# Intelligent-Microsystems-Lab/SNNQuantPrune

Hardware: AMD Instinct MI355X
Metric: samples/sec/node (DVS128 T=20, 4-bit/90%-pruned) (higher is better)
Workload: dtype fp6*fp4->f32 (integer-exact); 1 GPU; C3 topology: 3x(qconv3x3+BN+LIF+pool2) + qdense(32768->110)+LIF + vote, DVS128 128x128x2, T=20, bits 4/4/4/4, 90% pruned; batch_per_gpu=1024, global_batch=1024, frames=20, parallelism=dp1 (batch-sharded, all-gather logits)

## Files before the change

### include/snnqp.h

```cpp
#ifndef SNNQP_H_
#define SNNQP_H_

#include <stdint.h>

#ifdef __cplusplus
extern "C" {
#endif

typedef void *snnqp_stream_t;

enum {
  SNNQP_OK = 0,
  SNNQP_EINVAL = -1,
  SNNQP_EUNSUPPORTED = -2,
  SNNQP_EHIP = -3
};

enum { SNNQP_F32 = 0, SNNQP_U8 = 1, SNNQP_BITS = 2, SNNQP_EV1 = 3, SNNQP_EV4 = 4 };
enum { SNNQP_W_F32 = 0, SNNQP_W_I8 = 1 };
enum {
  SNNQP_NEURON_NONE = 0,
  SNNQP_NEURON_MULTI_STEP_LIF = 1,
  SNNQP_NEURON_PARAMETRIC_LEAKY_IF = 2,
  SNNQP_NEURON_LIF = 3
// ... 59 lines not shown
  int32_t H, W, Cin, Cout;
  int32_t KH, KW;
  int32_t stride_h, stride_w;
  int32_t pad_h_lo, pad_h_hi, pad_w_lo, pad_w_hi;
  int32_t in_dil_h, in_dil_w;
  int32_t k_dil_h, k_dil_w;
  int32_t groups;
} snnqp_conv_geom_t;

typedef struct {
  int32_t D, H, W, Cin, Cout;
  int32_t KD, KH, KW;
  int32_t stride[3];
  int32_t pad_lo[3], pad_hi[3];
  int32_t in_dil[3];
  int32_t k_dil[3];
  int32_t groups;
} snnqp_conv3d_geom_t;

#define SNNQP_VERSION 505
int snnqp_version(void);
const char *snnqp_last_error(void);
const char *snnqp_build_flags(void);

int snnqp_conv_out_shape(const snnqp_conv_geom_t *g, int32_t *OH, int32_t *OW);

int snnqp_quantize(int kind, const float *w, const float *mask, int64_t n,
                   int bits, float p0, float p1, float *fq_out,
                   int8_t *codes_out, int32_t *flags, snnqp_stream_t stream);
int snnqp_quantize_ex(int kind, const float *w, const float *mask, int64_t n,
                      int bits, int sign, float p0, float p1, float *fq_out,
                      int8_t *codes_out, int32_t *flags, snnqp_stream_t stream);

int snnqp_pack_codes_mfma(const int8_t *w, int64_t K, int32_t N, int32_t Npad,
                          int8_t *wt, snnqp_stream_t stream);

int snnqp_pack_codes_fp6(const int8_t *w, int64_t K, int32_t N, int32_t Npad, void *wt6,
                         snnqp_stream_t stream);

int snnqp_inspect_f32(const float *x, int64_t n, int32_t *flags,
                      snnqp_stream_t stream);
int snnqp_inspect_u8(const uint8_t *x, int64_t n, int32_t *flags,
                     snnqp_stream_t stream);
int snnqp_f32_to_u8(const float *x, uint8_t *y, int64_t n,
                    snnqp_stream_t stream);
int snnqp_narrow_f32(const float *x, uint8_t *y, int64_t n, int32_t *flags,
// ... 176 lines not shown
```

### snnquantprune_amd/_lib.py

```python

from __future__ import annotations

import ctypes
import os
from ctypes import (POINTER, Structure, c_char_p, c_float, c_int, c_int8,
                    c_int32, c_uint32, c_int64, c_void_p)

_HERE = os.path.dirname(os.path.abspath(__file__))
LIB_PATH = os.path.join(_HERE, "csrc", "libsnnqp.so")

ABI_VERSION = 505

F32, U8, BITS, EV1, EV4 = 0, 1, 2, 3, 4
W_F32, W_I8 = 0, 1
NEURON_NONE, NEURON_MULTI_STEP_LIF, NEURON_PARAMETRIC_LEAKY_IF, NEURON_LIF = 0, 1, 2, 3
SURR_FAST_SIGMOID, SURR_ATAN, SURR_SLAYER, SURR_SMOOTH_STEP, SURR_PIECEWISE_LINEAR = 0, 1, 2, 3, 4
Q_DUQ, Q_UNIFORM_STATIC, Q_PARAMETRIC_D, Q_PARAMETRIC_D_XMAX = 0, 1, 2, 3
IMPL_AUTO, IMPL_GENERIC, IMPL_MFMA = 0, 1, 2
FLAG_CODE_OVERFLOW, FLAG_MASK_NOT_BINARY = 1, 2
FLAG_NOT_INTEGER, FLAG_GT_ONE, FLAG_GT_127, FLAG_GT_15 = 4, 8, 16, 32
OK, EINVAL, EUNSUPPORTED, EHIP = 0, -1, -2, -3
STATUS_QUEUE_CORRUPT, STATUS_TICKET, STATUS_BOUND = 1, 2, 4


# ... 13 lines not shown

class NeuronT(Structure):
  _fields_ = [("kind", c_int32), ("k", c_float), ("v_threshold", c_float),
              ("v_reset", c_float), ("decay", c_void_p)]


class ConvGeomT(Structure):
  _fields_ = [(n, c_int32) for n in (
      "H", "W", "Cin", "Cout", "KH", "KW", "stride_h", "stride_w",
      "pad_h_lo", "pad_h_hi", "pad_w_lo", "pad_w_hi",
      "in_dil_h", "in_dil_w", "k_dil_h", "k_dil_w", "groups")]


class Conv3dGeomT(Structure):
  _fields_ = ([(n, c_int32) for n in ("D", "H", "W", "Cin", "Cout", "KD", "KH", "KW")]
              + [(n, c_int32 * 3) for n in ("stride", "pad_lo", "pad_hi", "in_dil", "k_dil")]
              + [("groups", c_int32)])


_PROTOTYPES = {
    "snnqp_version": (c_int, []),
    "snnqp_last_error": (c_char_p, []),
    "snnqp_build_flags": (c_char_p, []),
    "snnqp_conv_out_shape": (c_int, [POINTER(ConvGeomT), POINTER(c_int32),
                                     POINTER(c_int32)]),
    "snnqp_quantize": (c_int, [c_int, c_void_p, c_void_p, c_int64, c_int, c_float,
                               c_float, c_void_p, c_void_p, c_void_p, c_void_p]),
    "snnqp_quantize_ex": (c_int, [c_int, c_void_p, c_void_p, c_int64, c_int, c_int, c_float,
                                  c_float, c_void_p, c_void_p, c_void_p, c_void_p]),
    "snnqp_pack_codes_mfma": (c_int, [c_void_p, c_int64, c_int32, c_int32, c_void_p,
                                      c_void_p]),
    "snnqp_pack_codes_fp6": (c_int, [c_void_p, c_int64, c_int32, c_int32, c_void_p, c_void_p]),
    "snnqp_inspect_f32": (c_int, [c_void_p, c_int64, c_void_p, c_void_p]),
    "snnqp_inspect_u8": (c_int, [c_void_p, c_int64, c_void_p, c_void_p]),
    "snnqp_f32_to_u8": (c_int, [c_void_p, c_void_p, c_int64, c_void_p]),
    "snnqp_narrow_f32": (c_int, [c_void_p, c_void_p, c_int64, c_void_p, c_void_p]),
    "snnqp_pack_frames": (c_int, [c_void_p, c_int64, c_int32, c_int32, c_int, c_void_p, c_void_p,
                                  c_void_p]),
    "snnqp_unpack_frames": (c_int, [c_void_p, c_int, c_int64, c_int32, c_int32, c_void_p,
                                    c_void_p]),
    "snnqp_pack_bits": (c_int, [c_void_p, c_int, c_int64, c_int32, c_void_p,
                                c_void_p]),
    "snnqp_pack_bits_checked": (c_int, [c_void_p, c_int, c_int64, c_int32, c_void_p, c_void_p,
                                        c_void_p]),
    "snnqp_unpack_bits": (c_int, [c_void_p, c_int64, c_int32, c_void_p, c_void_p]),
    "snnqp_conv_forward": (c_int, [c_void_p, c_int, c_int64, POINTER(ConvGeomT),
# ... 143 lines not shown
```

### snnquantprune_amd/csrc/api.hip

```cpp
#include "common.h"

namespace snnqp {

static thread_local std::string g_last_error;

void set_error(const char *fmt, ...) {
  char buf[512];
  va_list ap;
  va_start(ap, fmt);
  vsnprintf(buf, sizeof(buf), fmt, ap);
  va_end(ap);
  g_last_error = buf;
}

}

extern "C" {

int snnqp_version(void) { return SNNQP_VERSION; }

const char *snnqp_last_error(void) { return snnqp::g_last_error.c_str(); }

#ifndef SNNQP_BUILD_FLAGS
#define SNNQP_BUILD_FLAGS ""
#endif
const char *snnqp_build_flags(void) { return SNNQP_BUILD_FLAGS; }

int snnqp_conv_out_shape(const snnqp_conv_geom_t *g, int32_t *OH, int32_t *OW) {
  SNNQP_REQUIRE(g && OH && OW, SNNQP_EINVAL, "conv_out_shape: null argument");
  SNNQP_REQUIRE(g->stride_h > 0 && g->stride_w > 0 && g->in_dil_h > 0 &&
                    g->in_dil_w > 0 && g->k_dil_h > 0 && g->k_dil_w > 0 &&
                    g->KH > 0 && g->KW > 0,
                SNNQP_EINVAL, "conv_out_shape: non-positive stride/dilation/kernel");
  const int64_t hd = g->H > 0 ? (int64_t)(g->H - 1) * g->in_dil_h + 1 : 0;
  const int64_t wd = g->W > 0 ? (int64_t)(g->W - 1) * g->in_dil_w + 1 : 0;
  const int64_t kh = (int64_t)(g->KH - 1) * g->k_dil_h + 1;
  const int64_t kw = (int64_t)(g->KW - 1) * g->k_dil_w + 1;
  const int64_t th = hd + g->pad_h_lo + g->pad_h_hi;
  const int64_t tw = wd + g->pad_w_lo + g->pad_w_hi;
  *OH = th < kh ? 0 : (int32_t)((th - kh) / g->stride_h + 1);
  *OW = tw < kw ? 0 : (int32_t)((tw - kw) / g->stride_w + 1);
  return SNNQP_OK;
}

}
```

### snnquantprune_amd/csrc/conv3x3_bits.hip

```cpp
#include <type_traits>

#include "conv_tile.h"

namespace snnqp {

typedef int v8i __attribute__((ext_vector_type(8)));
typedef float v16f __attribute__((ext_vector_type(16)));
typedef __attribute__((address_space(3))) const v4i lds_cv4i_t;
typedef __attribute__((address_space(3))) const uint32_t lds_cu32_t;

constexpr int F6_PITCH = HPITCH;
constexpr int F6_ROWS = 6;
constexpr int F6_NT = 256;
constexpr int F6_PLANE = F6_ROWS * HPITCH * 32;
constexpr int F6_NBUF = 3;
constexpr int F6_TAB = 256 * 32 * 4;
constexpr int DQT_BYTES = 16384;

__device__ __forceinline__ uint32_t fp6_codes4(uint32_t x) {
  const uint32_t m1 = (x >> 7) & 0x01010101u;
  const uint32_t mag = (x ^ (m1 * 0xFFu)) + m1;
  const uint32_t code = __builtin_amdgcn_perm(0x1E1C1A18u, 0x14100800u, mag);
  return code | (m1 << 5);
}

__device__ __forceinline__ uint32_t squeeze6(uint32_t c) {
  return (c & 0x3Fu) | ((c >> 2) & 0xFC0u) | ((c >> 4) & 0x3F000u) | ((c >> 6) & 0xFC0000u);
}

__device__ __forceinline__ void fp6_pack32(const v4i &lo, const v4i &hi, int (&d)[6]) {
  uint32_t t[8];
#pragma unroll
  for (int i = 0; i < 4; ++i) {
    t[i] = squeeze6(fp6_codes4((uint32_t)lo[i]));
    t[4 + i] = squeeze6(fp6_codes4((uint32_t)hi[i]));
  }
#pragma unroll
  for (int g = 0; g < 2; ++g) {
    d[3 * g + 0] = (int)(t[4 * g] | (t[4 * g + 1] << 24));
    d[3 * g + 1] = (int)((t[4 * g + 1] >> 8) | (t[4 * g + 2] << 16));
    d[3 * g + 2] = (int)((t[4 * g + 2] >> 16) | (t[4 * g + 3] << 8));
  }
}

enum { FMT_FP6 = 0, FMT_I8 = 1 };

constexpr int F6_WR_SLOT = 2;
constexpr int F6_BAR_SLOT = 4;
constexpr int F6_PF = 4;

__host__ __device__ constexpr int pair_tap(int p, int h) { return p < 3 ? p + 3 * h : 2 * p + h; }

template <int FMT, int CIN, int NF, bool POOL, int DQ, bool FMA = false, bool BNF = false, bool BNU = false>
__global__ void __launch_bounds__(F6_NT, 2)
conv3x3_bits_kernel(ConvMfmaArgs a) {
  static_assert(CIN == 32 || CIN == 64 || CIN == 96 || CIN == 128, "one to four 32-channel groups");
  static_assert(!BNU || (BNF && DQ == DQ_TABLE), "the uniform multiplier folds into the shared table");
  static_assert(DQ == DQ_ARITH || DQ == DQ_ONE || DQ == DQ_TABLE, "dequantisation mode");
  constexpr bool I8 = FMT == FMT_I8;
  constexpr bool TABLE = DQ == DQ_TABLE;
  static_assert(!(TABLE && I8), "the table is addressed by a float32 accumulator");
  typedef typename std::conditional<I8, v16i, v16f>::type acc_t;
  constexpr int BR = I8 ? 4 : 6;
  constexpr int WPP = CIN / 32;
  constexpr int NP = I8 ? WPP : (WPP + 1) / 2;
  constexpr int NPL = I8 ? WPP : WPP / 2;
  constexpr int PAIRS = I8 || WPP % 2 == 0 ? 0 : 5;
  constexpr int KS = 9 * NPL + PAIRS;
  constexpr int NPD = NPL > 0 ? NPL : 1;
  constexpr int HALO_B = NP * F6_PLANE;
  constexpr int FL = POOL ? 16 : 4;
  constexpr int SLOTS = 2 * FL;
  constexpr int NPIX = OutStage<POOL>::NPIX / 2;
  constexpr int TAB_OFF = F6_NBUF * HALO_B;
  constexpr int OB_OFF = TAB_OFF + (I8 ? 0 : F6_TAB);
  constexpr int DQT_OFF = OB_OFF + SLOTS * NPIX * 16 + 16;
  __shared__ __attribute__((aligned(128))) uint8_t lds[DQT_OFF + (TABLE ? DQT_BYTES : 0)];
  uint32_t *nxt = (uint32_t *)(lds + OB_OFF + SLOTS * NPIX * 16);
  uint32_t *obuf = (uint32_t *)(lds + OB_OFF);
  const uint32_t lds0 = lds_addr(lds) & 0x3FFFFu;

  const int tid = threadIdx.x, lane = tid & 63, wave = tid >> 6;
  const int n = lane & 31, h = lane >> 5;
  const int cg = wave & 3;
  const int cout_base = blockIdx.y * 128 + cg * 32;
  const bool wave_on = cout_base < a.Cout;
  const int cout = wave_on ? cout_base + n : n;
  const int cpar = cout < a.Cout ? cout : a.Cout - 1;
  const uint32_t cmask = chan_mask(cout_base, a.Cout);

  if (!I8) {
    for (int i = tid; i < 256 * 32; i += F6_NT) {
      const int e = i >> 5;
      uint32_t v = 0;
#pragma unroll
      for (int bit = 0; bit < 8; ++bit) v |= ((e >> bit) & 1) ? (0x2u << (4 * bit)) : 0u;
      ((uint32_t *)(lds + TAB_OFF))[i] = v;
    }
  }
  int bf[KS][BR];
  {
    const v4i *wtile = (const v4i *)a.wt + (int64_t)(cout_base >> 5) * (9 * WPP) * 64;
#pragma unroll
    for (int ks = 0; ks < KS; ++ks) {
      if constexpr (I8) {
        const v4i t = wave_on ? wtile[ks * 64 + lane] : v4i{0, 0, 0, 0};
        bf[ks][0] = t.x; bf[ks][1] = t.y; bf[ks][2] = t.z; bf[ks][3] = t.w;
      } else {
        const int ptap = pair_tap(ks - 9 * NPL, h);
        const bool pair = ks >= 9 * NPL;
        const int ks8 = pair ? ptap * WPP + WPP - 1 : (ks / NPD) * WPP + (ks % NPD) * 2 + h;
        v4i lo = {0, 0, 0, 0}, hi = {0, 0, 0, 0};
        if (wave_on && !(pair && ptap >= 9)) {
          lo = wtile[ks8 * 64 + n];
          hi = wtile[ks8 * 64 + 32 + n];
        }
        fp6_pack32(lo, hi, bf[ks]);
      }
    }
  }

  const uint32_t dqt_mid = lds0 + (uint32_t)DQT_OFF + 4u * (uint32_t)(TABLE ? a.lut_bound : 0);
  const float chain0 = TABLE ? __uint_as_float(dqt_mid) : 0.0f;
  if (TABLE) {
    const float mul0 = (BNU && a.bn.mul) ? a.bn.mul[0] : 1.0f;
    for (int i = tid; i <= 2 * a.lut_bound; i += F6_NT) {
      const float af = (float)(i - a.lut_bound);
      const float q = __builtin_fmaf(af, a.dq.rL, af * a.dq.rLlo);
      const float cur = q * a.dq.m;
      ((float *)(lds + DQT_OFF))[i] = BNU ? cur * mul0 : cur;
    }
  }

  LaneConsts lc = {0.f, 1.f, 0.f, 0.f, a.nrn.vr};
  if (a.bn.mean) { lc.bmean = a.bn.mean[cpar]; lc.bmul = a.bn.mul[cpar]; lc.bbias = a.bn.bias[cpar]; }
  if (a.nrn.kind == SNNQP_NEURON_LIF) lc.dec = a.nrn.decay[cpar];

  constexpr int SCALE_A = TABLE ? 64 : 127;
  constexpr int SCALE_B = TABLE ? 43 : 127;

  const int ty = ((n >> 2) & 1) | ((n >> 4) << 1);
  const int tx = (n & 3) | (((n >> 3) & 1) << 2);
  const uint32_t pixb = lds0 + (uint32_t)((ty * F6_PITCH + tx) * 32);
  const uint32_t abase_even = pixb + (uint32_t)((h ^ (ty & 1)) * 16);
  const uint32_t abase_odd = pixb + (uint32_t)((h ^ (ty & 1) ^ 1) * 16);
  const uint32_t abase_pv = pixb + (uint32_t)(h * F6_PITCH * 32 + ((ty ^ h) & 1) * 16);
  const uint32_t abase_ph = pixb + (uint32_t)(h * 32 + (ty & 1) * 16);
  struct Bases { uint32_t e, o, pv, ph; };

  const int s_pix = tid / WPP, s_wi = tid % WPP;
  const bool s_task = tid < F6_ROWS * HALO * WPP;
  const int wpm = (a.Cin + 31) >> 5;
  const int s_hy = s_pix / HALO, s_hx = s_pix % HALO;
  const uint32_t s_dst = lds0 + (uint32_t)((I8 ? s_wi : s_wi >> 1) * F6_PLANE +
                                           (s_hy * F6_PITCH + s_hx) * 32 +
                                           ((((I8 ? 0 : s_wi) & 1) ^ (s_hy & 1)) * 16));
  const uint32_t tabl = lds0 + TAB_OFF + (uint32_t)(lane & 31) * 4;
  const uint32_t *xb = (const uint32_t *)a.x;

  const int ob = out_pix<POOL>(0, lane) * 4 + cg;
  const bool store_lane = POOL ? lane < 8 : lane < 32;

  lds_barrier();

  acc_t cblk = {0, 0, 0, 0, 0, 0, 0, 0, 0, 0, 0, 0, 0, 0, 0, 0};
  if constexpr (TABLE) {
#pragma unroll
    for (int i = 0; i < 16; ++i) cblk[i] = chain0;
    asm volatile("" : "+v"(cblk));
  }
  PatchWalk pw(a);
  int r = __builtin_amdgcn_readfirstlane((int)pw.first);
  uint32_t processed = 0;
  while (r < (int)pw.count) {
    ++processed;
    int claimed = 0;
    if (pw.queue && tid == 0) claimed = (int)pw.claim();
    int b, y0, x0;
    pw.decode(a, r, b, y0, x0);

    float u[16];
    if (a.u0 && wave_on) {
      u_io_tile<true>(u, a, b, y0, x0, cout, h, 0);
    } else {
#pragma unroll
      for (int i = 0; i < 16; ++i) u[i] = 0.0f;
    }

    const int gy = y0 + s_hy - 1, gx = x0 + s_hx - 1;
    const bool s_valid = s_task && s_wi < wpm && gy >= 0 && gy < a.H && gx >= 0 && gx < a.W;
    const int64_t s_goff = (int64_t)b * a.xs_b + ((int64_t)gy * a.W + gx) * wpm + s_wi;
    uint32_t stgq[2] = {0, 0}, stg_cur = 0;
    auto stage_load = [&](int t, int par) {
      stgq[par] = s_valid ? xb[(int64_t)t * a.xs_t + s_goff] : 0u;
    };
    v4i s_exp = {0, 0, 0, 0};
    auto stage_expand = [&](int par) {
      if (I8) {
        stg_cur = stgq[par];
      } else if (s_task) {
        const uint32_t sw = stgq[par];
        s_exp.x = (int)*(lds_cu32_t *)(uintptr_t)(((sw & 0xFFu) << 7) + tabl);
        s_exp.y = (int)*(lds_cu32_t *)(uintptr_t)((((sw >> 8) & 0xFFu) << 7) + tabl);
        s_exp.z = (int)*(lds_cu32_t *)(uintptr_t)((((sw >> 16) & 0xFFu) << 7) + tabl);
        s_exp.w = (int)*(lds_cu32_t *)(uintptr_t)(((sw >> 24) << 7) + tabl);
      }
    };
    auto stage_write = [&](uint32_t bufoff) {
      typedef __attribute__((address_space(3))) v4i lds_v4i_t;
      if (I8) {
        if (s_task) {
          const uint32_t d = s_dst + bufoff;
          *(lds_v4i_t *)(uintptr_t)d = expand16<false>(stg_cur & 0xFFFFu);
          *(lds_v4i_t *)(uintptr_t)(s_hy & 1 ? d - 16 : d + 16) = expand16<false>(stg_cur >> 16);
        }
      } else if (s_task) {
        *(lds_v4i_t *)(uintptr_t)(s_dst + bufoff) = s_exp;
      }
    };
    auto a_read = [&](const Bases &ib, int ks) -> v4i {
      if (ks >= 9 * NPL) {
        const int p = ks - 9 * NPL;
        const uint32_t off = (uint32_t)(NPL * F6_PLANE + (p < 3 ? p : 2 * F6_PITCH + 2 * (p - 3)) * 32);
        return *(lds_cv4i_t *)(uintptr_t)((p < 3 ? ib.pv : ib.ph) + off);
      }
      const int tap = ks / NPD;
      const uint32_t off = (uint32_t)((ks % NPD) * F6_PLANE + ((tap / 3) * F6_PITCH + tap % 3) * 32);
      return *(lds_cv4i_t *)(uintptr_t)(((tap / 3) & 1 ? ib.o : ib.e) + off);
    };
    auto mfma_acc = [&](int ks, const v4i &av, const acc_t &c) -> acc_t {
      if constexpr (I8) {
        return __builtin_amdgcn_mfma_i32_32x32x32_i8(
            av, v4i{bf[ks][0], bf[ks][1], bf[ks][2], bf[ks][3]}, c, 0, 0, 0);
      } else {
        return __builtin_amdgcn_mfma_scale_f32_32x32x64_f8f6f4(
            v8i{av.x, av.y, av.z, av.w, 0, 0, 0, 0},
            v8i{bf[ks][0], bf[ks][1], bf[ks][2], bf[ks][3], bf[ks][4], bf[ks][5], 0, 0}, c,
            4 , 2 , 0, SCALE_A, 0, SCALE_B);
      }
    };
    const acc_t zero16 = {0, 0, 0, 0, 0, 0, 0, 0, 0, 0, 0, 0, 0, 0, 0, 0};
    auto dequant1 = [&](auto a0) -> float {
      if constexpr (TABLE) return *(lds_cfloat_t *)(uintptr_t)__float_as_uint((float)a0);
// ... 68 lines not shown
          word_insert(e, 6);
          word_combine(e, 7);
          word_insert(e, 7);
        }
      }
    };
    auto estage_head = [&](acc_t &accC, ETmp &e) {
      e.ew = 0;
#pragma unroll
      for (int g = 0; g < GP; ++g) e.ex[g][0] = e.ex[g][1] = e.euu[g][0] = e.euu[g][1] = 0.f;
#pragma unroll
      for (int j = 0; j < EYN; ++j) e.ey[j][0] = e.ey[j][1] = 0.f;
#pragma unroll
      for (int j = 0; j < YD; ++j) {
        e.ey[j][0] = dequant1(accC[2 * j]);
        e.ey[j][1] = dequant1(accC[2 * j + 1]);
      }
    };
    constexpr int NSTAGES = 8 * NST;
    auto store_word = [&](int t, uint32_t ew) {
      if (store_lane) obuf[(t % SLOTS) * (NPIX * 4) + ob] = ew & cmask;
    };

    constexpr int RING = KS % 6 == 0 && !TABLE ? 6 : KS % 3 == 0 ? 3 : KS % 7 == 0 ? 7 : KS;
    constexpr int PF = RING == 6 || (RING == 7 && !TABLE) ? F6_PF : 2;
    static_assert(KS % RING == 0 && PF < RING, "ring indices must repeat every step");
    v4i A[RING];

    constexpr bool LATE = TABLE || I8;
    constexpr int BAR_LATE = KS * 5 / 6 < KS - PF ? KS * 5 / 6 : KS - PF - 1;
    constexpr int WR_LATE = KS * 5 / 9 < BAR_LATE ? KS * 5 / 9 : BAR_LATE - 1;
    constexpr int WR_SLOT = LATE ? WR_LATE : F6_WR_SLOT < KS - PF - 2 ? F6_WR_SLOT : 1;
    constexpr int BAR_SLOT = LATE ? BAR_LATE : F6_BAR_SLOT < KS - PF ? F6_BAR_SLOT : WR_SLOT + 1;
    static_assert(WR_SLOT < BAR_SLOT && BAR_SLOT < KS - PF,
                  "the halo is written before the barrier, the next step's fragments read after it");
    constexpr int TAB_OPS = [] {
      int n = 0;
      if (TABLE)
        for (int st = (WR_SLOT + 1) * (8 * NST) / KS; st < (BAR_SLOT + 1) * (8 * NST) / KS; ++st)
          if ((st % (NST * GP)) / GP == 0) {
            const int j = (st / (NST * GP)) * GP + (st % (NST * GP)) % GP;
            if (j + YD < 8) n += 2;
          }
      return n;
    }();
    auto fused_step = [&](acc_t &accN, acc_t &accC, int s, const Bases &rd, const Bases &rn,
                          uint32_t wr_off, int par, bool more) {
      if (s + 2 < a.T) stage_expand(par);
      if (s + 4 < a.T) stage_load(s + 4, par);
      ETmp e;
      estage_head(accC, e);
#pragma unroll
      for (int ks = 0; ks < KS; ++ks) {
        if (ks == 0) accN = mfma_acc(0, A[0], TABLE ? cblk : zero16);
        else accN = mfma_acc(ks, A[ks % RING], accN);
        __builtin_amdgcn_sched_barrier(0);
        if (ks + PF < KS) A[(ks + PF) % RING] = a_read(rd, ks + PF);
        else if (more) A[(ks + PF) % RING] = a_read(rn, ks + PF - KS);
        {
          const int lo = ks * NSTAGES / KS, hi = (ks + 1) * NSTAGES / KS;
#pragma unroll
          for (int st = lo; st < hi; ++st) estage(accC, st, e);
        }
        if (ks == WR_SLOT && s + 2 < a.T) stage_write(wr_off);
        if (ks == BAR_SLOT) {
          constexpr int BAR_WAIT = BAR_SLOT - WR_SLOT + TAB_OPS < 15 ? BAR_SLOT - WR_SLOT + TAB_OPS : 15;
          asm volatile("s_waitcnt lgkmcnt(%0)\n\ts_barrier" : : "n"(BAR_WAIT) : "memory");
          if (s >= FL && s % FL == 0)
            flush_ring<POOL, SLOTS, F6_NT, NPIX>(obuf, a, s - FL, FL, b, y0, x0, tid);
        }
        asm volatile("" : "+v"(accN), "+v"(e.ew));
#pragma unroll
        for (int g = 0; g < GP; ++g)
          asm volatile("" : "+v"(e.ex[g][0]), "+v"(e.ex[g][1]), "+v"(e.euu[g][0]), "+v"(e.euu[g][1]));
        if constexpr (!TABLE) {
#pragma unroll
          for (int g = 0; g < EYN; ++g) asm volatile("" : "+v"(e.ey[g][0]), "+v"(e.ey[g][1]));
        }
        __builtin_amdgcn_sched_barrier(0);
      }
      store_word(s, e.ew);
    };
    auto epilogue = [&](acc_t &acc, int t) {
      ETmp e;
      estage_head(acc, e);
#pragma unroll
      for (int st = 0; st < NSTAGES; ++st) estage(acc, st, e);
      store_word(t, e.ew);
    };

    auto img = [&](int k) {
      const uint32_t d = (uint32_t)(k * HALO_B);
      return Bases{abase_even + d, abase_odd + d, abase_pv + d, abase_ph + d};
    };

    acc_t accA, accB;
    stage_load(0, 0);
    if (a.T > 1) stage_load(1, 1);
    stage_expand(0);
    if (a.T > 2) stage_load(2, 0);
    stage_write(0u);
    if (a.T > 1) {
      stage_expand(1);
      if (a.T > 3) stage_load(3, 1);
      stage_write((uint32_t)HALO_B);
    }
    lds_barrier();
    if (pw.queue && tid == 0) nxt[0] = (uint32_t)claimed;
    {
      const Bases i0 = img(0), i1 = img(1);
#pragma unroll
      for (int i = 0; i < PF; ++i) A[i] = a_read(i0, i);
#pragma unroll
      for (int ks = 0; ks < KS; ++ks) {
        if (ks == 0) accA = mfma_acc(0, A[0], TABLE ? cblk : zero16);
        else accA = mfma_acc(ks, A[ks % RING], accA);
        if (ks + PF < KS) A[(ks + PF) % RING] = a_read(i0, ks + PF);
        else if (a.T > 1) A[(ks + PF) % RING] = a_read(i1, ks + PF - KS);
        __builtin_amdgcn_sched_barrier(0);
      }
    }

    int s = 0;
    int k1 = 1, k2 = 2;
    for (; s + 2 < a.T; s += 2) {
      fused_step(accB, accA, s, img(k1), img(k2), (uint32_t)(k2 * HALO_B), 0, true);
      const int k3 = k1 == 0 ? 2 : k1 - 1;
      fused_step(accA, accB, s + 1, img(k2), img(k3), (uint32_t)(k3 * HALO_B), 1, s + 3 < a.T);
      k1 = k3;
      k2 = k3 == 2 ? 0 : k3 + 1;
    }
    if (s + 1 < a.T) {
      fused_step(accB, accA, s, img(k1), img(k2), (uint32_t)(k2 * HALO_B), 0, false);
      epilogue(accB, s + 1);
    } else {
      epilogue(accA, s);
    }
    lds_barrier();
    {
      const int done = a.T >= 2 ? ((a.T - 2) / FL) * FL : 0;
      flush_ring<POOL, SLOTS, F6_NT, NPIX>(obuf, a, done, a.T - done, b, y0, x0, tid);
    }
    if (a.u_out && wave_on) u_io_tile<false>(u, a, b, y0, x0, cout, h, 0);
    int r_next = r + (int)pw.stride;
    if (pw.queue) r_next = __builtin_amdgcn_readfirstlane((int)nxt[0]);
    r = r_next;
  }
  if (pw.queue && tid == 0) pw.finish(processed, a.npatch, a.status);
}

template <int FMT, int CIN, int NF, int DQ, bool FMA, bool BNF, bool BNU = false>
static void launch_bits_pool(const ConvMfmaArgs &a, bool pool, unsigned gy, hipStream_t st) {
  if (pool) launch_persistent(conv3x3_bits_kernel<FMT, CIN, NF, true, DQ, FMA, BNF, BNU>, a, gy, st, 0, F6_NT);
  else launch_persistent(conv3x3_bits_kernel<FMT, CIN, NF, false, DQ, FMA, BNF, BNU>, a, gy, st, 0, F6_NT);
}

template <int FMT, int CIN>
static void launch_bits_nf(const ConvMfmaArgs &a, int nf, bool pool, int dq, bool fma, bool bnf,
                           unsigned gy, hipStream_t st) {
  if (nf == NF_MUL) return launch_bits_pool<FMT, CIN, NF_MUL, DQ_ARITH, false, false>(a, pool, gy, st);
  if (nf == NF_DIV) return launch_bits_pool<FMT, CIN, NF_DIV, DQ_ARITH, false, false>(a, pool, gy, st);
  if (nf == NF_DECAY) return launch_bits_pool<FMT, CIN, NF_DECAY, DQ_ARITH, false, false>(a, pool, gy, st);
  if constexpr (FMT == FMT_FP6) {
    if (dq == DQ_TABLE) {
      if (fma && bnf && (a.bn.flags & SNNQP_BN_MUL_UNIFORM))
        return launch_bits_pool<FMT, CIN, NF_MUL0, DQ_TABLE, true, true, true>(a, pool, gy, st);
      if (fma && bnf) return launch_bits_pool<FMT, CIN, NF_MUL0, DQ_TABLE, true, true>(a, pool, gy, st);
      if (fma) return launch_bits_pool<FMT, CIN, NF_MUL0, DQ_TABLE, true, false>(a, pool, gy, st);
      if (bnf) return launch_bits_pool<FMT, CIN, NF_MUL0, DQ_TABLE, false, true>(a, pool, gy, st);
      return launch_bits_pool<FMT, CIN, NF_MUL0, DQ_TABLE, false, false>(a, pool, gy, st);
    }
    if (dq == DQ_ONE) {
      if (fma && bnf) return launch_bits_pool<FMT, CIN, NF_MUL0, DQ_ONE, true, true>(a, pool, gy, st);
      if (fma) return launch_bits_pool<FMT, CIN, NF_MUL0, DQ_ONE, true, false>(a, pool, gy, st);
      if (bnf) return launch_bits_pool<FMT, CIN, NF_MUL0, DQ_ONE, false, true>(a, pool, gy, st);
      return launch_bits_pool<FMT, CIN, NF_MUL0, DQ_ONE, false, false>(a, pool, gy, st);
    }
  }
  if (fma && bnf) return launch_bits_pool<FMT, CIN, NF_MUL0, DQ_ARITH, true, true>(a, pool, gy, st);
  if (fma) return launch_bits_pool<FMT, CIN, NF_MUL0, DQ_ARITH, true, false>(a, pool, gy, st);
  if (bnf) return launch_bits_pool<FMT, CIN, NF_MUL0, DQ_ARITH, false, true>(a, pool, gy, st);
  launch_bits_pool<FMT, CIN, NF_MUL0, DQ_ARITH, false, false>(a, pool, gy, st);
}

template <int FMT>
static void launch_bits_cin(const ConvMfmaArgs &a, int cin_pad, int nf, bool pool, int dq, bool fma,
                            bool bnf, unsigned gy, hipStream_t st) {
  if (cin_pad == 32) launch_bits_nf<FMT, 32>(a, nf, pool, dq, fma, bnf, gy, st);
  else if (cin_pad == 64) launch_bits_nf<FMT, 64>(a, nf, pool, dq, fma, bnf, gy, st);
  else if (cin_pad == 96) launch_bits_nf<FMT, 96>(a, nf, pool, dq, fma, bnf, gy, st);
  else launch_bits_nf<FMT, 128>(a, nf, pool, dq, fma, bnf, gy, st);
}

void launch_conv3x3_bits(const ConvMfmaArgs &a0, int cin_pad, bool i8, int nf, bool pool, int dq,
                         bool fma, bool bnf, unsigned gy, hipStream_t st) {
  ConvMfmaArgs a = a0;
  a.patch_h = 4;
  a.tiles_y = (a.H + 3) / 4;
  a.npatch = (int64_t)a.B * a.tiles_y * a.tiles_x;
  if (i8) launch_bits_cin<FMT_I8>(a, cin_pad, nf, pool, dq, fma, bnf, gy, st);
  else launch_bits_cin<FMT_FP6>(a, cin_pad, nf, pool, dq, fma, bnf, gy, st);
}

}
```

### snnquantprune_amd/csrc/conv3x3_u8c2.hip

```cpp
#include <atomic>
#include <map>
#include <mutex>
#include <tuple>
#include <type_traits>
#include <utility>

#include <vector>

#include "conv_tile.h"

namespace snnqp {

constexpr int HROW2 = 24;
constexpr int HCOPY2 = HALO * HROW2;
constexpr int HCONST2 = 2 * HCOPY2;
constexpr int HIMG2 = 496;
constexpr int TCHUNK = 32;
constexpr int U8C2_WPS = 4;
constexpr int STG_N = TCHUNK / 2;

typedef int v2i_a4 __attribute__((ext_vector_type(2), aligned(4)));
typedef __attribute__((address_space(3))) const v2i_a4 lds_cv2i_t;

__host__ __device__ inline int u8c2_table_bytes(int lutm, int bound, int rows) {
// ... 692 lines not shown
  do {                                                                             \
    if (pl) SNNQP_CONV_LAUNCH_IN(KERN, NFV, true, LM, LDS);                         \
    else SNNQP_CONV_LAUNCH_IN(KERN, NFV, false, LM, LDS);                           \
  } while (0)
#define SNNQP_CONV_LAUNCH(KERN, LM, LDS)                                           \
  do {                                                                             \
    if (nf == NF_MUL0) SNNQP_CONV_LAUNCH_NF(KERN, NF_MUL0, LM, LDS);                \
    else if (nf == NF_MUL) SNNQP_CONV_LAUNCH_NF(KERN, NF_MUL, LM, LDS);             \
    else if (nf == NF_DIV) SNNQP_CONV_LAUNCH_NF(KERN, NF_DIV, LM, LDS);             \
    else SNNQP_CONV_LAUNCH_NF(KERN, NF_DECAY, LM, LDS);                             \
  } while (0)
  if (in_type == SNNQP_BITS) {
    const bool fma = nf == NF_MUL0 && w->min_current_bits != 0 && w->abs_sum_max > 0 &&
                     lif_fma_is_exact(w->min_current_bits, a.nrn.k_log2, T, u0 != nullptr);
    const bool i8 = !(w->code_max > 0 && w->code_max <= 7);
    int dq = conv3x3_bits_dequant_form(w, nrn);
    if (dq == DQ_TABLE && !dq_table_trusted(stream_device(st), st)) dq = DQ_ARITH;
    const bool tab = dq == DQ_TABLE;
    const bool bnf = (a.bn.flags & (SNNQP_BN_MEAN_ZERO | SNNQP_BN_BIAS_ZERO)) ==
                     (SNNQP_BN_MEAN_ZERO | SNNQP_BN_BIAS_ZERO);
    a.lut_bound = tab ? (int32_t)w->abs_sum_max : 0;
    if (tab) check_code_bound_once(stream_device(st), (const int8_t *)w->w, (int64_t)9 * g->Cin, g->Cout,
                                   w->abs_sum_max, st);
    launch_conv3x3_bits(a, cin_pad, i8, nf, pl, dq, fma, bnf, gy, st);
  } else {
    const int lm = lutc ? LUT_CHANNEL : lut ? LUT_SHARED : LUT_NONE;
    if (lut) check_code_bound_once(stream_device(st), (const int8_t *)w->w, (int64_t)9 * g->Cin, g->Cout,
                                   w->abs_sum_max, st);
    const size_t lds_rest = lds_fixed - (size_t)a.tchunk * HIMG2 + u8c2_table_bytes(lm, a.lut_bound, a.lut_rows);
    for (int wgs = 4; wgs >= 2; --wgs) {
      const size_t per_wg = (size_t)(160 * 1024) / wgs - 512;
      int tc = a.tchunk;
      while (tc > 16 && (size_t)tc * HIMG2 + lds_rest > per_wg) tc -= 1;
      if ((size_t)tc * HIMG2 + lds_rest <= per_wg) {
        a.tchunk = tc;
        break;
      }
    }
    const size_t ldsb = (size_t)a.tchunk * HIMG2 + lds_rest;
    const bool one = !a.u0 && !a.u_out && a.T <= a.tchunk;
    if (lutc) SNNQP_CONV_LAUNCH(conv3x3_u8c2_kernel, LUT_CHANNEL, ldsb);
    else if (lut) SNNQP_CONV_LAUNCH(conv3x3_u8c2_kernel, LUT_SHARED, ldsb);
    else SNNQP_CONV_LAUNCH(conv3x3_u8c2_kernel, LUT_NONE, ldsb);
  }
#undef SNNQP_CONV_LAUNCH
#undef SNNQP_CONV_LAUNCH_NF
#undef SNNQP_CONV_LAUNCH_IN
// ... 53 lines not shown
```

### snnquantprune_amd/csrc/conv_tile.h

```cpp
#pragma once
#include "kernels.h"

namespace snnqp {


typedef int v4i __attribute__((ext_vector_type(4)));
typedef int v16i __attribute__((ext_vector_type(16)));
struct v2f {
  float x, y;
};
__device__ __forceinline__ v2f operator+(v2f a, v2f b) { return v2f{a.x + b.x, a.y + b.y}; }
__device__ __forceinline__ v2f operator-(v2f a, v2f b) { return v2f{a.x - b.x, a.y - b.y}; }
__device__ __forceinline__ v2f operator*(v2f a, v2f b) { return v2f{a.x * b.x, a.y * b.y}; }
__device__ __forceinline__ v2f operator+(v2f a, float b) { return v2f{a.x + b, a.y + b}; }
__device__ __forceinline__ v2f operator-(v2f a, float b) { return v2f{a.x - b, a.y - b}; }
__device__ __forceinline__ v2f operator*(v2f a, float b) { return v2f{a.x * b, a.y * b}; }
__device__ __forceinline__ v2f operator-(v2f a) { return v2f{-a.x, -a.y}; }
__device__ __forceinline__ v2f fma2(v2f a, v2f b, v2f c) {
  return v2f{__builtin_fmaf(a.x, b.x, c.x), __builtin_fmaf(a.y, b.y, c.y)};
}


enum { LUT_NONE = 0, LUT_SHARED = 1, LUT_CHANNEL = 2 };
constexpr int LUT_CAP = 4095;
// ... 424 lines not shown
int stream_device(hipStream_t st);

template <typename K>
static inline void launch_persistent(K kernel, ConvMfmaArgs a, unsigned gy, hipStream_t st,
                                     size_t dyn_lds = 0, int threads = 256) {
  int dev = 0, cus = 256, occ = 2, slot = -1;
  a.sched = gy <= (unsigned)SCHED_Y ? sched_acquire(st, &dev, &slot) : nullptr;
  if (!a.sched) dev = stream_device(st);
  a.status = a.sched ? device_status_word(dev) : nullptr;
  persistent_limits((const void *)kernel, threads, dyn_lds, dev, &cus, &occ);
  const int64_t gmax = (int64_t)cus * occ;
  unsigned gx = (unsigned)(a.npatch < gmax ? a.npatch : gmax);
  a.xcd_split = 0;
  if (gx >= 64 && a.B >= 8) {
    gx &= ~7u;
    a.xcd_split = 1;
  }
  hipLaunchKernelGGL(kernel, dim3(gx, gy), dim3(threads), dyn_lds, st, a);
  if (a.sched) sched_release(dev, slot, st);
}

enum { DQ_ARITH = 1, DQ_ONE = 2, DQ_TABLE = 3 };
constexpr int DQT_MAXA = 2047;
void launch_conv3x3_bits(const ConvMfmaArgs &a, int cin_pad, bool i8, int nf, bool pool, int dq,
                         bool fma, bool bnf, unsigned gy, hipStream_t st);

}
```

### snnquantprune_amd/linen.py

```python

from __future__ import annotations

import dataclasses
import functools
import hashlib
import math
import threading
from collections.abc import MutableMapping
from typing import Any, Callable, Dict, Iterable, Optional, Sequence

import torch

_tls = threading.local()


def _stack():
  if not hasattr(_tls, "stack"):
    _tls.stack = []
  return _tls.stack


class ConfigDict(MutableMapping):

  def __init__(self, *args, **kwargs):
# ... 64 lines not shown

_CHANNEL_COMPACTION = True


def set_channel_compaction(enabled: bool):
  global _CHANNEL_COMPACTION
  _CHANNEL_COMPACTION = bool(enabled)


def channel_compaction() -> bool:
  return _CHANNEL_COMPACTION


_CONV_KPACK = True


def set_conv_kpack(enabled: bool):
  global _CONV_KPACK
  _CONV_KPACK = bool(enabled)


def conv_kpack() -> bool:
  return _CONV_KPACK


def check_compute_dtype(dtype, who: str):
  global _dtype_warned
  if dtype in (torch.float32, None, "float32"):
    return
  if _DTYPE_POLICY == "float32":
    if not _dtype_warned:
      import sys
      print("snnquantprune_amd: %s asked for %r; computing in float32 (nn.set_compute_dtype_policy)"
            % (who, dtype), file=sys.stderr)
      _dtype_warned = True
    return
  raise NotImplementedError(
      "%s computes in float32 (got %r); nn.set_compute_dtype_policy('float32') runs such a "
      "request in float32 instead of refusing it" % (who, dtype))




def _default_device():
  return torch.device("cuda") if torch.cuda.is_available() else torch.device("cpu")

# ... 418 lines not shown
```

### snnquantprune_amd/ops.py

```python

from __future__ import annotations

import ctypes
from dataclasses import dataclass
from typing import Optional, Sequence, Tuple

import torch

from . import _lib as L




class PackedSpikes:

  def __init__(self, bits: torch.Tensor, channels: int):
    assert bits.dtype == torch.int32 and bits.is_contiguous()
    assert bits.shape[-1] == (channels + 31) // 32
    self.bits = bits
    self.channels = int(channels)
    self.flat_perm = None
    self.chan_map = None

  @property
# ... 123 lines not shown

  def device_index(self, device) -> torch.Tensor:
    key = str(device)
    t = self._dev.get(key)
    if t is None:
      t = self._dev[key] = torch.from_numpy(self.index.astype("int32")).to(device)
    return t

  def __repr__(self):
    return "ChannelMap(%d of %d, %d live)" % (self.index.size, self.full, int(self.live.sum()))


def scatter_spike_channels(s: "PackedSpikes", channel_map: torch.Tensor, cout: int) -> "PackedSpikes":
  bits = s.bits.contiguous()
  _require_gpu(bits, channel_map)
  assert channel_map.dtype == torch.int32 and channel_map.numel() == s.channels
  cw = (int(cout) + 31) // 32
  npix = bits.numel() // max(bits.shape[-1], 1) if bits.ndim else 0
  out = torch.empty(tuple(bits.shape[:-1]) + (cw,), dtype=torch.int32, device=bits.device)
  L.check(L.lib().snnqp_scatter_spike_channels(_ptr(bits), npix, s.channels,
                                                _ptr(channel_map.contiguous()), int(cout), _ptr(out),
                                                _stream()))
  return PackedSpikes(out, int(cout))


def expand_channels(x):
  cm = getattr(x, "chan_map", None)
  if cm is None:
    return x
  flat = x.flat_perm
  if flat is not None:
    c, h, w = flat
    lead = tuple(x.bits.shape[:-1])
    blk = PackedSpikes(x.bits.reshape(*lead, h, w, c // 32).contiguous(), c)
    full = scatter_spike_channels(blk, cm.device_index(x.device), cm.full)
    out = PackedSpikes(full.bits.reshape(*lead, h * w * ((cm.full + 31) // 32)), h * w * cm.full)
    out.flat_perm = (cm.full, h, w)
    return out
  return scatter_spike_channels(x, cm.device_index(x.device), cm.full)


def frame_units(H: int, W: int, fmt: int) -> int:
  return (H * W * 2 + 31) // 32 if fmt == L.EV1 else H * W


def pack_frames_host(x, fmt: int) -> PackedFrames:
# ... 1087 lines not shown
```

### snnquantprune_amd/spiking_learning.py

```python

from __future__ import annotations

import dataclasses
import math
from typing import Any, Callable, Optional

import numpy as np

import torch

from . import _lib as L
from . import linen as nn
from . import ops
from . import packing
from ._cache import TensorCache
from .flax_qconv import QuantConv
from .flax_qdense import QuantDense

Array = Any




def uniform(scale=1e-2, dtype=torch.float32):
# ... 271 lines not shown
      out = self._gated_block(u, inputs)
      if out is not None:
        return out
      inputs = inputs.to_dense()
    if isinstance(conn, QuantConv) and len(conn._ksize()) == 3:
      return self._conv3d_block(u, inputs)
    flat = getattr(inputs, "flat_perm", None)
    x, integer = packing.prepare_input(inputs)
    spec = integer is packing.SPECULATE
    if flat is not None:
      x.flat_perm = flat
    u0 = None if (u is None or isinstance(u, ZeroCarry)) else u
    tm = not self.batch_major_input
    is_dense = isinstance(conn, QuantDense)
    cmap_in = getattr(x, "chan_map", None)
    if cmap_in is not None:
      full_cin = cmap_in.full if flat is None else cmap_in.full * flat[1] * flat[2]
      pk = conn.packed_kernel(full_cin)
      if not (integer and pk.int_weight() is not None and is_dense == (flat is not None)
              and (is_dense or len(conn._ksize()) == 2)):
        x = ops.expand_channels(x)
        flat = x.flat_perm
        cmap_in = None
    cin = x.shape[-1]
    pk = conn.packed_kernel(cin if cmap_in is None else full_cin)
    packed_out = bool(integer) if self.packed is None else bool(self.packed)
    rows = None
    if cmap_in is not None:
      rows = cmap_in.index
      if flat is not None:
        hw = flat[1] * flat[2]
        rows = (rows[:, None] * hw + np.arange(hw)[None, :]).reshape(-1)
    cmap_out = None
    x_bound = self._input_bound(x)
    if (self.compact and nn.channel_compaction() and not is_dense and integer is True and u0 is None
        and not self.return_state and packed_out and len(conn._ksize()) == 2 and x_bound is not None
        and self.impl != L.IMPL_GENERIC and pk.int_weight() is not None):
      cmap_out = self._channel_plan(pk, self.neural_dynamics.neuron(conn.features),
                                    self.norm_fn.coeffs(conn.features) if self.norm_fn is not None else None,
                                    x_bound, cmap_in)
    if rows is not None or cmap_out is not None:
      pk = pk.sliced(rows, None if cmap_out is None else cmap_out.index)
    w = None
    if integer:
      if is_dense:
        n_pad = (conn.features + 31) // 32 * 32
# ... 350 lines not shown
```

Measured before the change: 94480 samples/s.

## Walk conv input channels in 16-channel halves to skip silent padding

When channel compaction leaves a live channel count that fits in one fewer 16-channel half group than the 32-padded width, the input spike tensor is truncated and the fp6 conv3x3 kernel is instantiated for CIN multiples of 16. The kernel gains extra K16 MFMA steps that pack the half group with the remaining taps, which removes MFMA work on always-zero padded channels. To support the new K-step counts it also generalises the register ring sizing and fixes the ring index used when prefetching the next step. A global toggle (on by default) controls the path. The cost is more template instantiations and more complex LDS addressing.

```diff
diff --git a/include/snnqp.h b/include/snnqp.h
--- a/include/snnqp.h
+++ b/include/snnqp.h
@@ -105,6 +105,8 @@
 int snnqp_version(void);
 const char *snnqp_last_error(void);
 const char *snnqp_build_flags(void);
+
+int snnqp_set_conv_k16(int enabled);
 
 int snnqp_conv_out_shape(const snnqp_conv_geom_t *g, int32_t *OH, int32_t *OW);
 
diff --git a/snnquantprune_amd/_lib.py b/snnquantprune_amd/_lib.py
--- a/snnquantprune_amd/_lib.py
+++ b/snnquantprune_amd/_lib.py
@@ -59,6 +59,7 @@
     "snnqp_version": (c_int, []),
     "snnqp_last_error": (c_char_p, []),
     "snnqp_build_flags": (c_char_p, []),
+    "snnqp_set_conv_k16": (c_int, [c_int]),
     "snnqp_conv_out_shape": (c_int, [POINTER(ConvGeomT), POINTER(c_int32),
                                      POINTER(c_int32)]),
     "snnqp_quantize": (c_int, [c_int, c_void_p, c_void_p, c_int64, c_int, c_float,
diff --git a/snnquantprune_amd/csrc/api.hip b/snnquantprune_amd/csrc/api.hip
--- a/snnquantprune_amd/csrc/api.hip
+++ b/snnquantprune_amd/csrc/api.hip
@@ -1,6 +1,11 @@
+#include <atomic>
+
 #include "common.h"
 
 namespace snnqp {
+
+static std::atomic<int> g_conv_k16{1};
+bool conv_k16_enabled() { return g_conv_k16.load(std::memory_order_relaxed) != 0; }
 
 static thread_local std::string g_last_error;
 
@@ -26,6 +31,11 @@
 #endif
 const char *snnqp_build_flags(void) { return SNNQP_BUILD_FLAGS; }
 
+int snnqp_set_conv_k16(int enabled) {
+  if (enabled < 0) return snnqp::conv_k16_enabled() ? 1 : 0;
+  return snnqp::g_conv_k16.exchange(enabled ? 1 : 0, std::memory_order_relaxed);
+}
+
 int snnqp_conv_out_shape(const snnqp_conv_geom_t *g, int32_t *OH, int32_t *OW) {
   SNNQP_REQUIRE(g && OH && OW, SNNQP_EINVAL, "conv_out_shape: null argument");
   SNNQP_REQUIRE(g->stride_h > 0 && g->stride_w > 0 && g->in_dil_h > 0 &&
diff --git a/snnquantprune_amd/csrc/conv3x3_bits.hip b/snnquantprune_amd/csrc/conv3x3_bits.hip
--- a/snnquantprune_amd/csrc/conv3x3_bits.hip
+++ b/snnquantprune_amd/csrc/conv3x3_bits.hip
@@ -4,6 +4,7 @@
 
 namespace snnqp {
 
+typedef int v2i __attribute__((ext_vector_type(2)));
 typedef int v8i __attribute__((ext_vector_type(8)));
 typedef float v16f __attribute__((ext_vector_type(16)));
 typedef __attribute__((address_space(3))) const v4i lds_cv4i_t;
@@ -50,11 +51,20 @@
 constexpr int F6_PF = 4;
 
 __host__ __device__ constexpr int pair_tap(int p, int h) { return p < 3 ? p + 3 * h : 2 * p + h; }
+__host__ __device__ constexpr int k16_tap(int q, int h, int i) { return i == 0 ? q + 3 * h : h == 0 ? 6 + q : 9; }
+
+constexpr bool ring_ok(int ks, int ring, int pf) {
+  if (pf >= ring || pf >= ks) return false;
+  for (int k = 0; k < ks; ++k)
+    for (int j = 1; j < pf; ++j)
+      if ((k + pf) % ks % ring == (k + j) % ks % ring) return false;
+  return true;
+}
 
 template <int FMT, int CIN, int NF, bool POOL, int DQ, bool FMA = false, bool BNF = false, bool BNU = false>
 __global__ void __launch_bounds__(F6_NT, 2)
 conv3x3_bits_kernel(ConvMfmaArgs a) {
-  static_assert(CIN == 32 || CIN == 64 || CIN == 96 || CIN == 128, "one to four 32-channel groups");
+  static_assert(CIN % 16 == 0 && CIN >= 16 && CIN <= 128, "one to eight 16-channel half groups");
   static_assert(!BNU || (BNF && DQ == DQ_TABLE), "the uniform multiplier folds into the shared table");
   static_assert(DQ == DQ_ARITH || DQ == DQ_ONE || DQ == DQ_TABLE, "dequantisation mode");
   constexpr bool I8 = FMT == FMT_I8;
@@ -62,11 +72,15 @@
   static_assert(!(TABLE && I8), "the table is addressed by a float32 accumulator");
   typedef typename std::conditional<I8, v16i, v16f>::type acc_t;
   constexpr int BR = I8 ? 4 : 6;
-  constexpr int WPP = CIN / 32;
+  constexpr int WPP = (CIN + 31) / 32;
+  constexpr int GW = CIN / 32;
+  constexpr bool HALF = CIN % 32 != 0;
   constexpr int NP = I8 ? WPP : (WPP + 1) / 2;
-  constexpr int NPL = I8 ? WPP : WPP / 2;
-  constexpr int PAIRS = I8 || WPP % 2 == 0 ? 0 : 5;
-  constexpr int KS = 9 * NPL + PAIRS;
+  constexpr int NPL = I8 ? GW : GW / 2;
+  constexpr int PAIRS = (I8 ? HALF : GW % 2 == 1) ? 5 : 0;
+  constexpr int PGRP = I8 ? GW : GW - 1;
+  constexpr int K16 = !I8 && HALF ? 3 : 0;
+  constexpr int KS = 9 * NPL + PAIRS + K16;
   constexpr int NPD = NPL > 0 ? NPL : 1;
   constexpr int HALO_B = NP * F6_PLANE;
   constexpr int FL = POOL ? 16 : 4;
@@ -104,12 +118,22 @@
 #pragma unroll
     for (int ks = 0; ks < KS; ++ks) {
       if constexpr (I8) {
-        const v4i t = wave_on ? wtile[ks * 64 + lane] : v4i{0, 0, 0, 0};
+        const int ptap = pair_tap(ks - 9 * NPL, h);
+        const bool pair = ks >= 9 * NPL;
+        const int idx = pair ? (ptap * WPP + GW) * 64 + n : ((ks / NPD) * WPP + ks % NPD) * 64 + lane;
+        const v4i t = wave_on && !(pair && ptap >= 9) ? wtile[idx] : v4i{0, 0, 0, 0};
         bf[ks][0] = t.x; bf[ks][1] = t.y; bf[ks][2] = t.z; bf[ks][3] = t.w;
+      } else if (ks >= 9 * NPL + PAIRS) {
+        const int q = ks - 9 * NPL - PAIRS;
+        const int t0 = k16_tap(q, h, 0), t1 = k16_tap(q, h, 1);
+        v4i lo = {0, 0, 0, 0}, hi = {0, 0, 0, 0};
+        if (wave_on) lo = wtile[(t0 * WPP + GW) * 64 + n];
+        if (wave_on && t1 < 9) hi = wtile[(t1 * WPP + GW) * 64 + n];
+        fp6_pack32(lo, hi, bf[ks]);
       } else {
         const int ptap = pair_tap(ks - 9 * NPL, h);
         const bool pair = ks >= 9 * NPL;
-        const int ks8 = pair ? ptap * WPP + WPP - 1 : (ks / NPD) * WPP + (ks % NPD) * 2 + h;
+        const int ks8 = pair ? ptap * WPP + PGRP : (ks / NPD) * WPP + (ks % NPD) * 2 + h;
         v4i lo = {0, 0, 0, 0}, hi = {0, 0, 0, 0};
         if (wave_on && !(pair && ptap >= 9)) {
           lo = wtile[ks8 * 64 + n];
@@ -146,7 +170,10 @@
   const uint32_t abase_odd = pixb + (uint32_t)((h ^ (ty & 1) ^ 1) * 16);
   const uint32_t abase_pv = pixb + (uint32_t)(h * F6_PITCH * 32 + ((ty ^ h) & 1) * 16);
   const uint32_t abase_ph = pixb + (uint32_t)(h * 32 + (ty & 1) * 16);
-  struct Bases { uint32_t e, o, pv, ph; };
+  const uint32_t abase_ka = pixb + (uint32_t)(h * F6_PITCH * 32 + (((GW ^ ty ^ h) & 1) * 16) +
+                                              (((ty + h) >> 1) & 1) * 8);
+  const uint32_t abase_kb = pixb + (uint32_t)((((GW ^ ty) & 1) * 16) + (((ty >> 1) & 1) ^ 1) * 8);
+  struct Bases { uint32_t e, o, pv, ph, ka, kb; };
 
   const int s_pix = tid / WPP, s_wi = tid % WPP;
   const bool s_task = tid < F6_ROWS * HALO * WPP;
@@ -156,6 +183,7 @@
                                            (s_hy * F6_PITCH + s_hx) * 32 +
                                            ((((I8 ? 0 : s_wi) & 1) ^ (s_hy & 1)) * 16));
   const uint32_t tabl = lds0 + TAB_OFF + (uint32_t)(lane & 31) * 4;
+  const uint32_t s_sh2 = K16 && s_wi == GW ? 0u : 16u, s_sh3 = K16 && s_wi == GW ? 8u : 24u;
   const uint32_t *xb = (const uint32_t *)a.x;
 
   const int ob = out_pix<POOL>(0, lane) * 4 + cg;
@@ -202,8 +230,13 @@
         const uint32_t sw = stgq[par];
         s_exp.x = (int)*(lds_cu32_t *)(uintptr_t)(((sw & 0xFFu) << 7) + tabl);
         s_exp.y = (int)*(lds_cu32_t *)(uintptr_t)((((sw >> 8) & 0xFFu) << 7) + tabl);
-        s_exp.z = (int)*(lds_cu32_t *)(uintptr_t)((((sw >> 16) & 0xFFu) << 7) + tabl);
-        s_exp.w = (int)*(lds_cu32_t *)(uintptr_t)(((sw >> 24) << 7) + tabl);
+        if constexpr (K16 > 0) {
+          s_exp.z = (int)*(lds_cu32_t *)(uintptr_t)((((sw >> s_sh2) & 0xFFu) << 7) + tabl);
+          s_exp.w = (int)*(lds_cu32_t *)(uintptr_t)((((sw >> s_sh3) & 0xFFu) << 7) + tabl);
+        } else {
+          s_exp.z = (int)*(lds_cu32_t *)(uintptr_t)((((sw >> 16) & 0xFFu) << 7) + tabl);
+          s_exp.w = (int)*(lds_cu32_t *)(uintptr_t)(((sw >> 24) << 7) + tabl);
+        }
       }
     };
     auto stage_write = [&](uint32_t bufoff) {
@@ -219,6 +252,14 @@
       }
     };
     auto a_read = [&](const Bases &ib, int ks) -> v4i {
+      if (ks >= 9 * NPL + PAIRS) {
+        typedef __attribute__((address_space(3))) const v2i lds_cv2i_t;
+        const int q = ks - 9 * NPL - PAIRS;
+        const uint32_t off = (uint32_t)((GW >> 1) * F6_PLANE + q * 32);
+        const v2i p0 = *(lds_cv2i_t *)(uintptr_t)(ib.ka + off);
+        const v2i p1 = *(lds_cv2i_t *)(uintptr_t)(ib.kb + off + 2 * F6_PITCH * 32);
+        return v4i{p0.x, p0.y, p1.x, p1.y};
+      }
       if (ks >= 9 * NPL) {
         const int p = ks - 9 * NPL;
         const uint32_t off = (uint32_t)(NPL * F6_PLANE + (p < 3 ? p : 2 * F6_PITCH + 2 * (p - 3)) * 32);
@@ -333,15 +374,16 @@
       if (store_lane) obuf[(t % SLOTS) * (NPIX * 4) + ob] = ew & cmask;
     };
 
-    constexpr int RING = KS % 6 == 0 && !TABLE ? 6 : KS % 3 == 0 ? 3 : KS % 7 == 0 ? 7 : KS;
-    constexpr int PF = RING == 6 || (RING == 7 && !TABLE) ? F6_PF : 2;
-    static_assert(KS % RING == 0 && PF < RING, "ring indices must repeat every step");
+    constexpr int RING_DIV = KS % 6 == 0 && !TABLE ? 6 : KS % 3 == 0 ? 3 : KS % 7 == 0 ? 7 : KS;
+    constexpr int RING = RING_DIV < KS || KS <= 5 ? RING_DIV : TABLE ? 3 : ring_ok(KS, 6, F6_PF) ? 6 : 8;
+    constexpr int PF = KS == 3 ? 1 : RING == 6 || RING == 8 || (RING == 7 && !TABLE) ? F6_PF : 2;
+    static_assert(ring_ok(KS, RING, PF), "a request must not overwrite a fragment still to be used");
     v4i A[RING];
 
     constexpr bool LATE = TABLE || I8;
     constexpr int BAR_LATE = KS * 5 / 6 < KS - PF ? KS * 5 / 6 : KS - PF - 1;
     constexpr int WR_LATE = KS * 5 / 9 < BAR_LATE ? KS * 5 / 9 : BAR_LATE - 1;
-    constexpr int WR_SLOT = LATE ? WR_LATE : F6_WR_SLOT < KS - PF - 2 ? F6_WR_SLOT : 1;
+    constexpr int WR_SLOT = LATE ? WR_LATE : F6_WR_SLOT < KS - PF - 2 ? F6_WR_SLOT : KS - PF > 2 ? 1 : 0;
     constexpr int BAR_SLOT = LATE ? BAR_LATE : F6_BAR_SLOT < KS - PF ? F6_BAR_SLOT : WR_SLOT + 1;
     static_assert(WR_SLOT < BAR_SLOT && BAR_SLOT < KS - PF,
                   "the halo is written before the barrier, the next step's fragments read after it");
@@ -367,7 +409,7 @@
         else accN = mfma_acc(ks, A[ks % RING], accN);
         __builtin_amdgcn_sched_barrier(0);
         if (ks + PF < KS) A[(ks + PF) % RING] = a_read(rd, ks + PF);
-        else if (more) A[(ks + PF) % RING] = a_read(rn, ks + PF - KS);
+        else if (more) A[(ks + PF - KS) % RING] = a_read(rn, ks + PF - KS);
         {
           const int lo = ks * NSTAGES / KS, hi = (ks + 1) * NSTAGES / KS;
 #pragma unroll
@@ -402,7 +444,7 @@
 
     auto img = [&](int k) {
       const uint32_t d = (uint32_t)(k * HALO_B);
-      return Bases{abase_even + d, abase_odd + d, abase_pv + d, abase_ph + d};
+      return Bases{abase_even + d, abase_odd + d, abase_pv + d, abase_ph + d, abase_ka + d, abase_kb + d};
     };
 
     acc_t accA, accB;
@@ -427,7 +469,7 @@
         if (ks == 0) accA = mfma_acc(0, A[0], TABLE ? cblk : zero16);
         else accA = mfma_acc(ks, A[ks % RING], accA);
         if (ks + PF < KS) A[(ks + PF) % RING] = a_read(i0, ks + PF);
-        else if (a.T > 1) A[(ks + PF) % RING] = a_read(i1, ks + PF - KS);
+        else if (a.T > 1) A[(ks + PF - KS) % RING] = a_read(i1, ks + PF - KS);
         __builtin_amdgcn_sched_barrier(0);
       }
     }
@@ -469,9 +511,11 @@
 template <int FMT, int CIN>
 static void launch_bits_nf(const ConvMfmaArgs &a, int nf, bool pool, int dq, bool fma, bool bnf,
                            unsigned gy, hipStream_t st) {
-  if (nf == NF_MUL) return launch_bits_pool<FMT, CIN, NF_MUL, DQ_ARITH, false, false>(a, pool, gy, st);
-  if (nf == NF_DIV) return launch_bits_pool<FMT, CIN, NF_DIV, DQ_ARITH, false, false>(a, pool, gy, st);
-  if (nf == NF_DECAY) return launch_bits_pool<FMT, CIN, NF_DECAY, DQ_ARITH, false, false>(a, pool, gy, st);
+  if constexpr (CIN % 32 == 0) {
+    if (nf == NF_MUL) return launch_bits_pool<FMT, CIN, NF_MUL, DQ_ARITH, false, false>(a, pool, gy, st);
+    if (nf == NF_DIV) return launch_bits_pool<FMT, CIN, NF_DIV, DQ_ARITH, false, false>(a, pool, gy, st);
+    if (nf == NF_DECAY) return launch_bits_pool<FMT, CIN, NF_DECAY, DQ_ARITH, false, false>(a, pool, gy, st);
+  }
   if constexpr (FMT == FMT_FP6) {
     if (dq == DQ_TABLE) {
       if (fma && bnf && (a.bn.flags & SNNQP_BN_MUL_UNIFORM))
@@ -495,22 +539,27 @@
 }
 
 template <int FMT>
-static void launch_bits_cin(const ConvMfmaArgs &a, int cin_pad, int nf, bool pool, int dq, bool fma,
+static void launch_bits_cin(const ConvMfmaArgs &a, int cin_walk, int nf, bool pool, int dq, bool fma,
                             bool bnf, unsigned gy, hipStream_t st) {
-  if (cin_pad == 32) launch_bits_nf<FMT, 32>(a, nf, pool, dq, fma, bnf, gy, st);
-  else if (cin_pad == 64) launch_bits_nf<FMT, 64>(a, nf, pool, dq, fma, bnf, gy, st);
-  else if (cin_pad == 96) launch_bits_nf<FMT, 96>(a, nf, pool, dq, fma, bnf, gy, st);
+  if (nf != NF_MUL0) cin_walk = (cin_walk + 31) / 32 * 32;
+  if (cin_walk == 16) launch_bits_nf<FMT, 16>(a, nf, pool, dq, fma, bnf, gy, st);
+  else if (cin_walk == 32) launch_bits_nf<FMT, 32>(a, nf, pool, dq, fma, bnf, gy, st);
+  else if (cin_walk == 48) launch_bits_nf<FMT, 48>(a, nf, pool, dq, fma, bnf, gy, st);
+  else if (cin_walk == 64) launch_bits_nf<FMT, 64>(a, nf, pool, dq, fma, bnf, gy, st);
+  else if (cin_walk == 80) launch_bits_nf<FMT, 80>(a, nf, pool, dq, fma, bnf, gy, st);
+  else if (cin_walk == 96) launch_bits_nf<FMT, 96>(a, nf, pool, dq, fma, bnf, gy, st);
+  else if (cin_walk == 112) launch_bits_nf<FMT, 112>(a, nf, pool, dq, fma, bnf, gy, st);
   else launch_bits_nf<FMT, 128>(a, nf, pool, dq, fma, bnf, gy, st);
 }
 
-void launch_conv3x3_bits(const ConvMfmaArgs &a0, int cin_pad, bool i8, int nf, bool pool, int dq,
+void launch_conv3x3_bits(const ConvMfmaArgs &a0, int cin_walk, bool i8, int nf, bool pool, int dq,
                          bool fma, bool bnf, unsigned gy, hipStream_t st) {
   ConvMfmaArgs a = a0;
   a.patch_h = 4;
   a.tiles_y = (a.H + 3) / 4;
   a.npatch = (int64_t)a.B * a.tiles_y * a.tiles_x;
-  if (i8) launch_bits_cin<FMT_I8>(a, cin_pad, nf, pool, dq, fma, bnf, gy, st);
-  else launch_bits_cin<FMT_FP6>(a, cin_pad, nf, pool, dq, fma, bnf, gy, st);
-}
-
-}
+  if (i8) launch_bits_cin<FMT_I8>(a, cin_walk, nf, pool, dq, fma, bnf, gy, st);
+  else launch_bits_cin<FMT_FP6>(a, cin_walk, nf, pool, dq, fma, bnf, gy, st);
+}
+
+}
diff --git a/snnquantprune_amd/csrc/conv3x3_u8c2.hip b/snnquantprune_amd/csrc/conv3x3_u8c2.hip
--- a/snnquantprune_amd/csrc/conv3x3_u8c2.hip
+++ b/snnquantprune_amd/csrc/conv3x3_u8c2.hip
@@ -738,7 +738,9 @@
     a.lut_bound = tab ? (int32_t)w->abs_sum_max : 0;
     if (tab) check_code_bound_once(stream_device(st), (const int8_t *)w->w, (int64_t)9 * g->Cin, g->Cout,
                                    w->abs_sum_max, st);
-    launch_conv3x3_bits(a, cin_pad, i8, nf, pl, dq, fma, bnf, gy, st);
+    const int cin16 = (g->Cin + 15) / 16 * 16;
+    const int cin_walk = conv_k16_enabled() && cin16 + 16 == cin_pad ? cin16 : cin_pad;
+    launch_conv3x3_bits(a, cin_walk, i8, nf, pl, dq, fma, bnf, gy, st);
   } else {
     const int lm = lutc ? LUT_CHANNEL : lut ? LUT_SHARED : LUT_NONE;
     if (lut) check_code_bound_once(stream_device(st), (const int8_t *)w->w, (int64_t)9 * g->Cin, g->Cout,
diff --git a/snnquantprune_amd/csrc/conv_tile.h b/snnquantprune_amd/csrc/conv_tile.h
--- a/snnquantprune_amd/csrc/conv_tile.h
+++ b/snnquantprune_amd/csrc/conv_tile.h
@@ -470,7 +470,8 @@
 
 enum { DQ_ARITH = 1, DQ_ONE = 2, DQ_TABLE = 3 };
 constexpr int DQT_MAXA = 2047;
-void launch_conv3x3_bits(const ConvMfmaArgs &a, int cin_pad, bool i8, int nf, bool pool, int dq,
+void launch_conv3x3_bits(const ConvMfmaArgs &a, int cin_walk, bool i8, int nf, bool pool, int dq,
                          bool fma, bool bnf, unsigned gy, hipStream_t st);
-
-}
+bool conv_k16_enabled();
+
+}
diff --git a/snnquantprune_amd/linen.py b/snnquantprune_amd/linen.py
--- a/snnquantprune_amd/linen.py
+++ b/snnquantprune_amd/linen.py
@@ -110,6 +110,16 @@
 
 def conv_kpack() -> bool:
   return _CONV_KPACK
+
+
+def set_conv_k16(enabled: bool):
+  from . import _lib
+  _lib.lib().snnqp_set_conv_k16(1 if enabled else 0)
+
+
+def conv_k16() -> bool:
+  from . import _lib
+  return bool(_lib.lib().snnqp_set_conv_k16(-1))
 
 
 def check_compute_dtype(dtype, who: str):
diff --git a/snnquantprune_amd/ops.py b/snnquantprune_amd/ops.py
--- a/snnquantprune_amd/ops.py
+++ b/snnquantprune_amd/ops.py
@@ -169,6 +169,19 @@
                                                 _ptr(channel_map.contiguous()), int(cout), _ptr(out),
                                                 _stream()))
   return PackedSpikes(out, int(cout))
+
+
+def truncate_silent_channels(x: "PackedSpikes"):
+  cm = x.chan_map
+  n = max(16, (int(cm.live.sum()) + 15) // 16 * 16)
+  if n >= cm.index.size or (n + 31) // 32 != x.bits.shape[-1] or cm.live[n:].any():
+    return x, cm
+  cut = getattr(cm, "_cut16", None)
+  if cut is None:
+    cut = cm._cut16 = ChannelMap(cm.index[:n], cm.live[:n], cm.full)
+  out = PackedSpikes(x.bits, n)
+  out.chan_map = cut
+  return out, cut
 
 
 def expand_channels(x):
diff --git a/snnquantprune_amd/spiking_learning.py b/snnquantprune_amd/spiking_learning.py
--- a/snnquantprune_amd/spiking_learning.py
+++ b/snnquantprune_amd/spiking_learning.py
@@ -317,6 +317,8 @@
         x = ops.expand_channels(x)
         flat = x.flat_perm
         cmap_in = None
+      elif not is_dense:
+        x, cmap_in = ops.truncate_silent_channels(x)
     cin = x.shape[-1]
     pk = conn.packed_kernel(cin if cmap_in is None else full_cin)
     packed_out = bool(integer) if self.packed is None else bool(self.packed)
```

Result: faster. 96470 samples/s (median of 6 runs) (+2.1%).
